# simonkosina/vbt

Hardware: AMD Instinct MI355X
Metric: frames/sec end-to-end (detect+NMS+track), EfficientDet-Lite0 320x320 (higher is better)
Workload: dtype int8

## Files before the change

vbt_amd/csrc/detector.hip:

```cpp
#include <algorithm>
#include <cmath>
#include <chrono>
#include <functional>
#include <map>
#include <set>
#include <type_traits>
#include <tuple>

#include "launchers.h"

namespace vbt {

static thread_local char g_err[512] = "";
void set_error(const char* fmt, ...) {
  va_list ap;
  va_start(ap, fmt);
  vsnprintf(g_err, sizeof(g_err), fmt, ap);
  va_end(ap);
}

bool lds_opt_in(const void* fn, LdsOptIn* state) {
  int dev = 0;
  if (hipGetDevice(&dev) != hipSuccess || dev < 0 || dev >= 64) { set_error("lds_opt_in: no current HIP device"); return false; }
  if (state->dev[dev] > 0) return true;
// ... 320 lines not shown
};
static FusedPlan resolve_fused(const vbt_model* m, const Step& s, int variant, int B) {
  const FusedArgs& a = s.fa;
  const OpRec& dop = m->ops[s.d_op];
  const int k = dop.k, stride = dop.stride;
  const bool ex = s.family == F_MBCONV, ks12 = a.KSe == 1 || a.KSe == 2;
  int var = variant;
  if (var < 0) {
    var = ((m->flags & VBT_MODEL_IMAGE_BLOCKS) && !resolve_fused(m, s, 5, B).rc) ? 5 : ((m->flags & VBT_MODEL_CHUNK48) ? 9 : 1);
    const FusedPlan p17 = (m->flags & VBT_MODEL_TILE128) ? resolve_fused(m, s, 17, B) : FusedPlan{};
    if (!p17.rc && p17.L.ppw2) var |= 16;
  }
  const bool mdw = var & 1, half = var & 2;
  const bool nt3 = (var & 8) && mdw && a.nch3 > 0 && s.nbp <= 2 && a.KSe >= 1 && a.KSe <= 4;
  FusedPlan p;
  if (var & 4) {
    const int HW = a.H * a.W, OHW = a.OH * a.OW;
    if (!ex || HW > 400 || OHW > 400 || !s.ib.data) { p.refuse(VBT_ERR_ARG, "fused_mbconv: whole-image variant not applicable"); return p; }
    p.image = true;
    p.PH = std::max((a.OH - 1) * stride + k, a.pad_t + a.H);
    p.PW = std::max((a.OW - 1) * stride + k, a.pad_l + a.W);
    p.NB = (a.Cout + 63) / 64;
    const int NPGo = (OHW + 15) / 16;
    const int units = (NPGo * p.NB + IB_WAVES - 1) / IB_WAVES;
    p.maxu = units <= 2 ? 2 : units <= 3 ? 3 : 4;
    p.L.k = k; p.L.stride = stride; p.L.lds_bytes = ((HW * a.T0S + 15) & ~15) + p.PH * p.PW * FB_EST + NPGo * 16 * FB_DST + s.ib.bytes;
    if (units > 4 || p.L.lds_bytes > 160 * 1024 || s.ib.bytes > 16 * IB_NPF * IB_THREADS) p.refuse(VBT_ERR_ARG, "fused_mbconv: whole-image variant not applicable");
    return p;
  }
  p.TX = a.TX;
  p.TY = half && a.TY >= 2 ? (a.TY + 1) / 2 : a.TY;
  const bool ppw2 = (var & 16) && ex && mdw && ks12 && s.nbp <= 2 && !half;
  if (ppw2) { p.TX = 16; p.TY = 8; }
  const bool dw64 = ppw2 || (ex && mdw && a.wd64 && p.TX == 8 && p.TY == 8 && ks12 && s.nbp <= 2);
  const int est = !ex ? 0 : !nt3 ? FB_EST : dw64 ? 48 : 72;
  p.tiles_x = (a.OW + p.TX - 1) / p.TX;
  p.tiles_y = (a.OH + p.TY - 1) / p.TY;
  p.L = FusedLaunch{k, stride, s.nbp, ex, mdw, nt3, ppw2, dw64, fused_tile_lds(a, k, stride, p.TX, p.TY, est, ppw2 ? 2 : 1, s.nbp),
                    (unsigned)((long)B * p.tiles_x * p.tiles_y)};
  if (ppw2 && (a.OW < 16 || a.OH < 8 || !a.wd64)) p.refuse(VBT_ERR_ARG, "fused_mbconv: the 128-pixel variant needs maps of at least 16 x 8");
  else if (ppw2 && p.L.lds_bytes > 64 * 1024) p.refuse(VBT_ERR_ARG, "fused_mbconv: 128-pixel tile needs %d bytes of LDS", p.L.lds_bytes);
  return p;
}
static int launch_fused_step(const vbt_model* m, const Step& s, FusedArgs a, int B, hipStream_t st) {
  const FusedPlan p = resolve_fused(m, s, s.variant, B);
  if (p.rc) return p.report();
  if (p.image) return launch_mbconv_image(a, s.ib, p.L.k, p.L.stride, p.maxu, p.PW, p.PH, p.NB, p.L.lds_bytes, B, st);
  a.TX = p.TX; a.TY = p.TY; a.tiles_x = p.tiles_x; a.tiles_y = p.tiles_y;
  return launch_fused_block(a, p.L, st);
}

struct ExpDwLaunch : Verdict {
  bool second = false; int cpw = 1, nw = 0, gpw = 0, lds = 0; unsigned grid = 0;
};
static ExpDwLaunch resolve_expdw(const vbt_model*, const Step& s, int variant, int B) {
  static const int xd_force = getenv("VBT_XD_VARIANT") ? atoi(getenv("VBT_XD_VARIANT")) : -100;
// ... 260 lines not shown
    cand = {0};
    for (int r : {1, 2, 4, 8, 16})
      if (r <= m->tensors[op.output].h) cand.push_back(r);
    if (m->tensors[op.output].c % 8 == 0) { cand.push_back(100); cand.push_back(101); }
  } else if (st.family == F_PW && st.KS64 <= 4) {
    cand = {0, 1};
  } else if (st.family == F_PW) {
    cand = {-1, 2, 3, 4, 5, 6};
  } else if (is_fused_tile(st.family)) {
    cand = {0, 1, 3, 5};
    if (st.family == F_MBCONV && st.fa.nch3 > 0 && st.nbp <= 2 && st.fa.KSe >= 1 && st.fa.KSe <= 4) { cand.push_back(9); cand.push_back(11); }
    if (st.family == F_MBCONV && st.nbp <= 2 && (st.fa.KSe == 1 || st.fa.KSe == 2)) {
      cand.push_back(17);
      if (st.fa.nch3 > 0) cand.push_back(25);
    }
  } else if (st.family == F_MULTI) {
    cand = {0, 1};
  } else if (st.family == F_EXPDW) {
    cand.clear();
    for (int cpw : {1, 2, 3, 4, 6})
      if (cpw <= st.xd.nchunks) cand.push_back(cpw);
    if (st.xd2_ok)
      for (int cpw : {1, 2, 3, 4, 6})
        if (cpw <= st.xd.nchunks) {
          if (st.xd2_gpw > 0) cand.push_back(100 + cpw);
          if (st.xd2_gpw16 > 0) cand.push_back(200 + cpw);
        }
  } else if (st.family == F_BAND) {
    cand = {-1, 0, 1};
  }
// ... 46 lines not shown
  }
  (void)hipDeviceSynchronize();
}

static PlanShape plan_shape(const vbt_model* m) {
  PlanShape shape;
  for (const Group& g : m->groups) {
    std::vector<std::vector<PlanStepShape>> alts;
    for (const Alt& a : g.alts) {
      std::vector<PlanStepShape> steps;
      for (const Step& st : a.steps) {
        PlanStepShape ps;
        ps.family = kFamilyName[st.family];
        ps.variants = candidate_variants(m, st);
        auto add = [&](int v) { if (std::find(ps.variants.begin(), ps.variants.end(), v) == ps.variants.end()) ps.variants.push_back(v); };
        for (int v = 0; v < 32 && is_fused_tile(st.family); v++)
          if (variant_ok(m, st, v)) add(v);
        add(-1);
        add(st.variant);
        steps.push_back(ps);
      }
      alts.push_back(steps);
    }
    shape.groups.push_back(alts);
  }
  return shape;
}
static bool load_plan(vbt_model* m, const char* path) {
  const PlanShape shape = plan_shape(m);
  std::vector<PlanChoice> sel;
  std::string note;
// ... 630 lines not shown
```

vbt_amd/csrc/dev_common.h:

```cpp
#pragma once
#include "common.h"

namespace vbt {

typedef int v4i __attribute__((ext_vector_type(4)));

__device__ __forceinline__ int requant(int acc, float mult, int zp, int lo, int hi) {
  float t = (float)acc * mult;
  t = fminf(fmaxf(t, -65536.0f), 65536.0f);
  int q = (int)__builtin_rintf(t) + zp;
  return min(max(q, lo), hi);
}
__device__ __forceinline__ unsigned pack4(int a, int b, int c, int d) {
  return (unsigned)(a & 255) | ((unsigned)(b & 255) << 8) | ((unsigned)(c & 255) << 16) | ((unsigned)(d & 255) << 24);
}

struct Rq {
  float lo_f, hi_f, off;
  int full;
  int kb;
};
constexpr int RQ_KBIAS = 0x4B400000;
__host__ __device__ inline Rq make_rq(int zp, int lo, int hi, int kb = 0) {
  return Rq{(float)(lo - zp), (float)(hi - zp), (float)(zp + 128), (lo <= -128 && hi >= 127) ? 1 : 0, kb};
// ... 30 lines not shown
    v2f r0 = (t0 + magic) + back;
    v2f r1 = (t1 + magic) + back;
    return pack4_u8f(r0.x, r0.y, r1.x, r1.y);
  }
  v2f r0 = {__builtin_amdgcn_fmed3f(__builtin_rintf(t0.x), q.lo_f, q.hi_f), __builtin_amdgcn_fmed3f(__builtin_rintf(t0.y), q.lo_f, q.hi_f)};
  v2f r1 = {__builtin_amdgcn_fmed3f(__builtin_rintf(t1.x), q.lo_f, q.hi_f), __builtin_amdgcn_fmed3f(__builtin_rintf(t1.y), q.lo_f, q.hi_f)};
  r0 = r0 + off;
  r1 = r1 + off;
  return pack4_u8f(r0.x, r0.y, r1.x, r1.y);
}
__device__ __forceinline__ v4i diag_operand(unsigned wb, int i) {
  const unsigned sh = wb << (8 * (i & 3));
  const int d = i >> 2;
  return (v4i){d == 0 ? (int)sh : 0, d == 1 ? (int)sh : 0, d == 2 ? (int)sh : 0, d == 3 ? (int)sh : 0};
}
__device__ __forceinline__ int fdiv_small(int n, float rcp_d) { return (int)(((float)n + 0.5f) * rcp_d); }
__device__ __forceinline__ float frcp(int d) { return __builtin_amdgcn_rcpf((float)d); }
__device__ __forceinline__ v4i v4i_from(const int4& b) { return (v4i){b.x, b.y, b.z, b.w}; }
__device__ __forceinline__ int4 int4_plus(const int4& b, int k) { return make_int4(b.x + k, b.y + k, b.z + k, b.w + k); }
template <class F>
__device__ __forceinline__ void rq_dispatch(const Rq& q, F&& f) {
  if (q.kb) { if (q.full) f(std::integral_constant<int, 3>{}); else f(std::integral_constant<int, 2>{}); }
  else { if (q.full) f(std::integral_constant<int, 1>{}); else f(std::integral_constant<int, 0>{}); }
}

__device__ __forceinline__ unsigned rq_pack_i(const v4i& acc, const int4& b, const float4& mu, const Rq& q) {
  const v4i a2 = {acc[0] + b.x, acc[1] + b.y, acc[2] + b.z, acc[3] + b.w};
  return rq_pack_b(a2, mu, q);
}

// ... 52 lines not shown
```

vbt_amd/csrc/expdw2_block.h:

```cpp
#pragma once
#include <type_traits>

#ifdef VBT_XD_PROF
#define XD2_STAMP(k) do { if (tid == 0) a.prof[(long)blockIdx.x * 32 + (k)] = __builtin_amdgcn_s_memtime(); } while (0)
#else
#define XD2_STAMP(k) do { } while (0)
#endif


struct ExpDw2Args {
  const int8_t* x;
  int8_t* out;
  int H, W, Cin, OH, OW, Ce;
  int pad_t, pad_l;
  int nchunks, cpw;
  int nbands, brows;
  int XB;
  int EQS, EYS;
  int e_bytes;
  int PS;
  int pe_off;
  int pd_off;
  const v4i* pe;
  const v4i* pd;
  Rq rqe;
  unsigned zeb;
  Rq rqd;
#ifdef VBT_XD_PROF
  unsigned long long* prof;
#endif
};

__device__ __forceinline__ v4i toeplitz_operand(unsigned w4, int c) {
  const int sh = 8 * c;
  return (v4i){(int)((w4 & 0xffu) << sh), (int)(((w4 >> 8) & 0xffu) << sh), (int)(((w4 >> 16) & 0xffu) << sh), (int)((w4 >> 24) << sh)};
}

constexpr int XD2_NPG = 8;
template <int PG, class F, class FC>
__device__ __forceinline__ void d_pair(F& d_units, FC full_c, int NPGo) {
  if constexpr (PG < XD2_NPG) {
    if (PG + 1 < NPGo) d_units(full_c, std::integral_constant<int, 2>{}, std::integral_constant<int, PG>{});
    else if (PG < NPGo) d_units(full_c, std::integral_constant<int, 1>{}, std::integral_constant<int, PG>{});
    if (PG + 2 < NPGo) d_pair<PG + 2>(d_units, full_c, NPGo);
  }
}

template <int KK, int S, int KS64, int NW, int GPW>
__global__ __launch_bounds__(64 * NW) void expdw2_kernel(ExpDw2Args a) {
  constexpr int DY = S, DX = 4 / S;
  constexpr int XD2_THREADS = 64 * NW, HW2 = NW / 2, QW = 16 / NW;
// ... 188 lines not shown
```

vbt_amd/csrc/fused_block.h:

```cpp
#pragma once

struct FusedArgs {
  const int8_t* x;
  int8_t* out;
  int H, W, Cin, OH, OW, Cout;
  int pad_t, pad_l;
  int TX, TY, tiles_x, tiles_y;
  int T0S;
  int nchunks;
  int zx;
  const long* we;
  const int* be;
  const float* me;
  int KSe, ze, loe, hie;
  Rq rqe;
  const long* we3;
  const long* wdm3;
  const v4i* wp3;
  int nch3, KSp3;
  const float* wd;
  const int* bd;
  const float* md;
  int zd, lod, hid;
  Rq rqd;
  const long* wdm;
  const int* bdm;
  const v4i* wd64;
  const long* wd64c;
  const v4i* wp;
  const int* bp;
  const float* mp;
  int KSp, zo, lop, hip;
  Rq rqp;
  int has_res;
  AddQ resq;
  int n_src;
  const int8_t* src[3];
  int sh[3], sw[3], smode[3], spt[3], spl[3];
  int chain;
  AddQ sumq, preq;
};

__device__ __forceinline__ unsigned node_sum4(const unsigned u[3], const FusedArgs& a) {
// ... 4 lines not shown

typedef unsigned short v2u16 __attribute__((ext_vector_type(2)));
__device__ __forceinline__ unsigned pk_max_u16(unsigned a, unsigned b) {
  v2u16 x, y;
  __builtin_memcpy(&x, &a, 4);
  __builtin_memcpy(&y, &b, 4);
  v2u16 r = __builtin_elementwise_max(x, y);
  unsigned o;
  __builtin_memcpy(&o, &r, 4);
  return o;
}

constexpr int FB_EST = 80;
constexpr int FB_DST = 80;

template <int KK, int S, int NBP, bool EXPAND, bool MDW, int KSE = 0, int NT = 4, int PPW = 1, bool DW64 = false>
__device__ __forceinline__ void fused_block_body(const FusedArgs& a, int tile, unsigned char* fb_smem) {
  static_assert(PPW == 1 || MDW, "128-pixel tiles exist for the matrix-pipe depthwise only");
  static_assert(!DW64 || (EXPAND && MDW && (KK == 3 || KK == 5)), "DW64: fused expand blocks, 3x3 / 5x5");
  const int tid = threadIdx.x, wave = tid >> 6, lane = tid & 63, r = lane & 15, g = lane >> 4;
  const int trow = fdiv_small(tile, frcp(a.tiles_x));
  const int tx = tile - trow * a.tiles_x;
  const int bimg = fdiv_small(trow, frcp(a.tiles_y));
  const int ty = trow - bimg * a.tiles_y;
  const long b = bimg;
  const int oy0 = ty * a.TY, ox0 = tx * a.TX;
  const int TXp = (a.TX + 3) & ~3;
  const int HWx = (TXp - 1) * S + KK, HWy = (a.TY - 1) * S + KK, NPh = HWx * HWy;
  const int iy0 = oy0 * S - a.pad_t, ix0 = ox0 * S - a.pad_l;
  const float rcp_hwx = frcp(HWx), rcp_txp = frcp(TXp);
  unsigned char* T0 = fb_smem;
  unsigned char* E = T0 + ((NPh * a.T0S + 15) & ~15);
  constexpr int EST = (EXPAND && NT == 3) ? (DW64 ? 48 : 72) : FB_EST;
  unsigned char* D = E + (EXPAND ? ((NPh * EST + 15) & ~15) : 0);
  bool stage_p = false;
  if constexpr (!EXPAND && NBP <= 2) stage_p = a.nchunks == 1;
  unsigned char* WPS = D + 64 * PPW * FB_DST;
  unsigned char* BPS = WPS + NBP * 4096;

  bool summed = false;
  if constexpr (!EXPAND) summed = a.n_src > 0;
  if (summed) {
    const int nd = a.Cin >> 2;
    const unsigned zb4 = (unsigned)(a.zx & 255) * 0x01010101u;
    const int pstep = fdiv_small(256, frcp(nd));
    int p = fdiv_small(tid, frcp(nd));
    const int cd = tid - p * nd;
    const bool up2[3] = {a.H == 2 * a.sh[0] && a.W == 2 * a.sw[0], a.H == 2 * a.sh[1] && a.W == 2 * a.sw[1], a.H == 2 * a.sh[2] && a.W == 2 * a.sw[2]};
    for (; tid < pstep * nd && p < NPh; p += pstep) {
// ... 107 lines not shown
  const int nsx = TXp >> 2;
  const int sy = fdiv_small(strip, frcp(nsx)), sx = (strip - sy * nsx) * 4;
  const bool dw_active = sy < a.TY;
  int hbase[4 * PPW];
#pragma unroll
  for (int pg = 0; pg < 4 * PPW; pg++) hbase[pg] = 0;
  if constexpr (MDW && !DW64) {
#pragma unroll
    for (int pg = 0; pg < 4 * PPW; pg++) {
      int slot = pg * 16 + r;
      int sq = TXp == 8 ? (slot >> 3) : fdiv_small(slot, rcp_txp);
      int py_ = min(sq, a.TY - 1), px_ = slot - sq * TXp;
      hbase[pg] = (py_ * S) * HWx + px_ * S;
    }
  }
  constexpr int KTP = (KK * KK + 1) / 2;
  long wpre[KTP];
  int4 bpre = make_int4(0, 0, 0, 0);
  float4 mpre = make_float4(0.f, 0.f, 0.f, 0.f);
  if constexpr (!EXPAND && MDW) {
    const long* wm0 = a.wdm + ((long)wave * KTP) * 64 + lane;
#pragma unroll
    for (int mi = 0; mi < KTP; mi++) wpre[mi] = wm0[mi * 64];
    bpre = *(const int4*)(a.bdm + 16 * wave + 4 * g);
    mpre = *(const float4*)(a.md + 16 * wave + 4 * g);
  }
  __syncthreads();

  constexpr int CH = 16 * NT;
  const int nch = NT == 3 ? a.nch3 : a.nchunks;
  const long* const wdm_ = NT == 3 ? a.wdm3 : a.wdm;
  for (int c = 0; c < nch; c++) {
    constexpr bool PREF_DW = EXPAND && MDW && KSE >= 3;
    if constexpr (PREF_DW) {
      if (NT == 4 || wave < NT) {
        const long* wmc = wdm_ + ((long)(c * NT + wave) * KTP) * 64 + lane;
#pragma unroll
        for (int mi = 0; mi < KTP; mi++) wpre[mi] = wmc[mi * 64];
        bpre = *(const int4*)(a.bdm + c * CH + 16 * wave + 4 * g);
        mpre = *(const float4*)(a.md + c * CH + 16 * wave + 4 * g);
      }
    }
    if (EXPAND) {
      int4 eb[NT];
      float4 em[NT];
#pragma unroll
      for (int t = 0; t < NT; t++) {
        eb[t] = *(const int4*)(a.be + c * CH + 4 * NT * g + 4 * t);
        em[t] = *(const float4*)(a.me + c * CH + 4 * NT * g + 4 * t);
      }
      const unsigned zeb = (unsigned)(a.ze & 255) * 0x01010101u;
      const long* w = (NT == 3 ? a.we3 : a.we) + (long)c * a.KSe * NT * 64 + lane;
      long wreg[KSE > 0 ? KSE : 1][NT];
      if constexpr (KSE > 0) {
#pragma unroll
        for (int ks = 0; ks < KSE; ks++)
#pragma unroll
// ... 21 lines not shown
          } else {
#pragma unroll 2
            for (int ks = 0; ks < a.KSe; ks++) {
              long bv = *(const long*)(brow + 32 * ks);
#pragma unroll
              for (int t = 0; t < NT; t++) ea[t] = __builtin_amdgcn_mfma_i32_16x16x32_i8(w[(ks * NT + t) * 64], bv, ea[t], 0, 0, 0);
            }
          }
          unsigned d[NT];
#pragma unroll
          for (int t = 0; t < NT; t++) {
            d[t] = rq_pack_b<FULLK>(ea[t], em[t], a.rqe);
            if ((oob_mask >> i) & 1u) d[t] = zeb;
          }
          if (!((tail_mask >> i) & 1u)) {
            if constexpr (NT == 4) {
              *(uint4*)(E + p * FB_EST + 16 * g) = make_uint4(d[0], d[1], d[2], d[3]);
            } else {
#pragma unroll
              for (int t = 0; t < NT; t++) *(unsigned*)(E + p * EST + 4 * NT * g + 4 * t) = d[t];
            }
          }
        }
      };
      rq_dispatch(a.rqe, expand_loop);
      __syncthreads();
    }
    if constexpr (DW64) {
      constexpr int TXP = 8 * PPW, HWX = (TXP - 1) * S + KK;
      constexpr int KT64 = KK == 3 ? 3 : 7;
      constexpr int PGS = (16 / TXP) * S * HWX * EST;
      if (NT == 4 || wave < NT) {
        const unsigned long long wc = (unsigned long long)a.wd64c[(long)(c * NT + wave) * 64 + lane];
        v4i wreg[KT64];
#pragma unroll
        for (int mi = 0; mi < KT64; mi++) wreg[mi] = diag_operand((unsigned)(wc >> (8 * mi)) & 0xffu, r);
        const int4 bq0 = *(const int4*)(a.bdm + c * CH + 16 * wave + 4 * g);
        const float4 mum = *(const float4*)(a.md + c * CH + 16 * wave + 4 * g);
        const int hb = TXP == 8 ? ((r >> 3) * S * HWX + (r & 7) * S) : r * S;
        const unsigned char* baseH = E + hb * EST + 16 * wave + g * EST;
        const unsigned char* baseV = E + hb * EST + 16 * wave + g * (HWX * EST);
        auto dw_walk = [&](auto mode_tag) {
          constexpr int RM = decltype(mode_tag)::value;
// ... 91 lines not shown
        }
      }
      const int4 bq = *(const int4*)(a.bd + c * 64 + 4 * cq);
      const float4 mu = *(const float4*)(a.md + c * 64 + 4 * cq);
#pragma unroll
      for (int o = 0; o < 4; o++) {
        v4i ai = {(int)dacc[o][0], (int)dacc[o][1], (int)dacc[o][2], (int)dacc[o][3]};
        unsigned dd = rq_pack_i(ai, bq, mu, a.rqd);
        *(unsigned*)(D + (sy * TXp + sx + o) * FB_DST + 4 * cq) = dd;
      }
    }
    __syncthreads();
    {
      v4i bv[PPW];
#pragma unroll
      for (int pp = 0; pp < PPW; pp++) bv[pp] = *(const v4i*)(D + ((wave * PPW + pp) * 16 + r) * FB_DST + 16 * g);
#pragma unroll
      for (int nb = 0; nb < NBP; nb++) {
        const v4i* w = stage_p ? (const v4i*)WPS + (nb * 4) * 64 + lane
                               : (NT == 3 ? a.wp3 + ((long)(nb * a.KSp3 + c) * 4) * 64 : a.wp + ((long)(nb * a.KSp + c) * 4) * 64) + lane;
#pragma unroll
        for (int t = 0; t < 4; t++) {
          const v4i wv = w[t * 64];
#pragma unroll
          for (int pp = 0; pp < PPW; pp++) acc[pp][nb][t] = __builtin_amdgcn_mfma_i32_16x16x64_i8(wv, bv[pp], acc[pp][nb][t], 0, 0, 0);
        }
      }
    }
    if (!EXPAND && c + 1 < nch) __syncthreads();
  }

// ... 39 lines not shown
#pragma unroll
        for (int t = 0; t < 4; t++)
#pragma unroll
          for (int j = 0; j < 4; j++)
            if (c0 + 4 * t + j < a.Cout) o[4 * t + j] = (int8_t)(d[t] >> (8 * j));
      }
    }
  }
  }
}


#ifndef FB_MINW
#define FB_MINW 1
#endif
template <int KK, int S, int NBP, bool EXPAND, bool MDW, int KSE = 0, int NT = 4, int PPW = 1, bool DW64 = false>
__global__ __launch_bounds__(256, FB_MINW) void fused_block_kernel(FusedArgs a) {
  extern __shared__ __attribute__((aligned(16))) unsigned char fb_smem_dyn[];
  fused_block_body<KK, S, NBP, EXPAND, MDW, KSE, NT, PPW, DW64>(a, blockIdx.x, fb_smem_dyn);
}

struct MultiTiles {
  int n;
  int start[13];
};
template <int KK, int S, int NBP, bool EXPAND, bool MDW>
__global__ __launch_bounds__(256, FB_MINW) void fused_block_multi_kernel(const FusedArgs* __restrict__ args, MultiTiles mt) {
  extern __shared__ __attribute__((aligned(16))) unsigned char fb_smem_dyn[];
  int p = 0;
#pragma unroll
  for (int i = 1; i < 12; i++)
    if (i < mt.n && (int)blockIdx.x >= mt.start[i]) p = i;
  fused_block_body<KK, S, NBP, EXPAND, MDW>(args[p], (int)blockIdx.x - mt.start[p], fb_smem_dyn);
}
// ... 138 lines not shown
```

vbt_amd/csrc/k_fused_mbconv.hip:

```cpp
#include "launchers.h"

namespace vbt {

#define FB_P2(KK, S, NBP, KSE)                                                                                      \
  do {                                                                                                              \
    if (L.nt3) fused_block_kernel<KK, S, NBP, true, true, KSE, 3, 2, true><<<grid, 256, L.lds_bytes, st>>>(a);      \
    else fused_block_kernel<KK, S, NBP, true, true, KSE, 4, 2, true><<<grid, 256, L.lds_bytes, st>>>(a);            \
  } while (0)
#define FB_P2K(KK, S)                                                                                               \
  do {                                                                                                              \
    if (L.nbp == 1 && a.KSe == 1) FB_P2(KK, S, 1, 1);                                                               \
    else if (L.nbp == 1) FB_P2(KK, S, 1, 2);                                                                        \
    else if (a.KSe == 1) FB_P2(KK, S, 2, 1);                                                                        \
    else FB_P2(KK, S, 2, 2);                                                                                        \
  } while (0)
#define FB_DW64(KK, S, NBP)                                                                                                                    \
  do {                                                                                                                                         \
    if (L.nt3 && a.KSe == 1) fused_block_kernel<KK, S, (NBP <= 2 ? NBP : 1), true, true, 1, 3, 1, true><<<grid, 256, L.lds_bytes, st>>>(a);    \
    else if (L.nt3) fused_block_kernel<KK, S, (NBP <= 2 ? NBP : 1), true, true, 2, 3, 1, true><<<grid, 256, L.lds_bytes, st>>>(a);            \
    else if (a.KSe == 1) fused_block_kernel<KK, S, (NBP <= 2 ? NBP : 1), true, true, 1, 4, 1, true><<<grid, 256, L.lds_bytes, st>>>(a);       \
    else fused_block_kernel<KK, S, (NBP <= 2 ? NBP : 1), true, true, 2, 4, 1, true><<<grid, 256, L.lds_bytes, st>>>(a);                       \
  } while (0)
#define FB_LAUNCH(KK, S, NBP)                                                                                                                          \
  do {                                                                                                                                                 \
// ... 7 lines not shown
    else if (L.mdw && a.KSe == 3) fused_block_kernel<KK, S, NBP, true, true, 3><<<grid, 256, L.lds_bytes, st>>>(a);                                   \
    else if (L.mdw && a.KSe == 4) fused_block_kernel<KK, S, NBP, true, true, 4><<<grid, 256, L.lds_bytes, st>>>(a);                                   \
    else if (L.mdw) fused_block_kernel<KK, S, NBP, true, true><<<grid, 256, L.lds_bytes, st>>>(a);                                                    \
    else fused_block_kernel<KK, S, NBP, true, false><<<grid, 256, L.lds_bytes, st>>>(a);                                                              \
  } while (0)
#define FB_NBP(KK, S)                                      \
  do {                                                     \
    switch (L.nbp) {                                       \
      case 1: FB_LAUNCH(KK, S, 1); break;                  \
      case 2: FB_LAUNCH(KK, S, 2); break;                  \
      case 3: FB_LAUNCH(KK, S, 3); break;                  \
      default: FB_LAUNCH(KK, S, 5); break;                 \
    }                                                      \
  } while (0)

int launch_fused_mbconv(const FusedArgs& a, const FusedLaunch& L, hipStream_t st) {
  const dim3 grid(L.grid);
  if (L.ppw2) {
    if (L.k == 3 && L.stride == 1) FB_P2K(3, 1);
    else if (L.k == 3 && L.stride == 2) FB_P2K(3, 2);
    else if (L.k == 5 && L.stride == 1) FB_P2K(5, 1);
    else FB_P2K(5, 2);
    return VBT_OK;
  }
  if (L.k == 3 && L.stride == 1) FB_NBP(3, 1);
  else if (L.k == 3 && L.stride == 2) FB_NBP(3, 2);
  else if (L.k == 5 && L.stride == 1) FB_NBP(5, 1);
  else FB_NBP(5, 2);
  return VBT_OK;
}

// ... 2 lines not shown
```

vbt_amd/csrc/launchers.h:

```cpp
#pragma once
#include "dev_common.h"

namespace vbt {
#include "fused_block.h"
#include "stem_block.h"
#include "image_block.h"
#include "expdw_block.h"
#include "expdw2_block.h"
#include "band_block.h"

struct FusedLaunch {
  int k, stride, nbp;
  bool expand;
  bool mdw;
  bool nt3;
  bool ppw2;
  bool dw64;
  int lds_bytes;
  unsigned grid;
};
int launch_fused_block(const FusedArgs& a, const FusedLaunch& L, hipStream_t st);
int launch_fused_multi(const FusedArgs* d_args, const MultiTiles& mt, int k, int stride, int nbp, bool mdw, int lds_bytes, unsigned grid,
                       hipStream_t st);
int launch_dw_tile(const DwTileArgs& a, int k, int stride, bool mdw, dim3 grid, int lds_bytes, hipStream_t st);
int launch_mbconv_image(const FusedArgs& a, const ImageBundle& wb, int k, int stride, int maxu, int PW, int PH, int NB, int lds_bytes, int B,
                        hipStream_t st);
int launch_band_one(const BandArgs& a, bool chained, unsigned grid, int lds_bytes, hipStream_t st);
int launch_band_multi(const BandArgs* d_probs, const MultiTiles& mt, int C, bool chained, unsigned grid, int lds_bytes, hipStream_t st);
int launch_expdw(const ExpDwArgs& a, int k, int stride, int KS64, unsigned grid, int lds_bytes, hipStream_t st);
int launch_expdw2(const ExpDw2Args& a, int k, int stride, int KS64, int nw, int gpw, unsigned grid, int lds_bytes, hipStream_t st);
int launch_stem_block(const StemBlockArgs& a, bool full_range, unsigned grid, hipStream_t st);

}
```

vbt_amd/csrc/planner.h:

```cpp
#pragma once

static int conv_kb(const vbt_model* m, const OpRec& op) {
  const bool off = getenv("VBT_NO_KBIAS") != nullptr;
  if (off || (op.type != OP_STEM && op.type != OP_PW && op.type != OP_DW)) return 0;
  const TensorRec& tin = m->tensors[op.inputs[0]];
  const TensorRec& tout = m->tensors[op.output];
  const int8_t* w = (const int8_t*)(m->blob.data() + op.w_off);
  const int32_t* bq = (const int32_t*)(m->blob.data() + op.b_off);
  const bool dw = op.type == OP_DW;
  const int N = tout.c, K = dw ? op.k * op.k : op.k * op.k * tin.c;
  for (int co = 0; co < N; co++) {
    long long sa = 0;
    for (int k = 0; k < K; k++) sa += std::abs((int)(dw ? w[(size_t)k * N + co] : w[(size_t)co * K + k]));
    if (255 * sa + std::llabs((long long)bq[co]) >= (1ll << 22) - 1) return 0;
  }
  return 1;
}

static void choose_tile(int OH, int OW, int KK, int S, bool expand, int* TXo, int* TYo, int slots = 64) {
  double best = 1e300;
  for (int TX = 1; TX <= std::min(OW, 64); TX++) {
    int TXp = (TX + 3) & ~3;
    int TY = std::min(OH, slots / TXp);
    if (TY < 1) continue;
    int tiles = ((OW + TX - 1) / TX) * ((OH + TY - 1) / TY);
    int NPh = ((TXp - 1) * S + KK) * ((TY - 1) * S + KK);
    double cost = tiles * ((expand ? 1.0 : 0.35) * NPh + (double)slots);
    if (cost < best) { best = cost; *TXo = TX; *TYo = TY; }
  }
}

static int fused_tile_lds(const FusedArgs& a, int k, int stride, int TX, int TY, int est, int ppw, int nbp) {
  const int TXp = (TX + 3) & ~3;
  const int NPh = ((TXp - 1) * stride + k) * ((TY - 1) * stride + k);
  int lds = ((NPh * a.T0S + 15) & ~15) + ((NPh * est + 15) & ~15) + ppw * 64 * FB_DST;
  if (!est && a.nchunks == 1 && nbp <= 2) lds += nbp * (4096 + 512);
  return lds;
}

struct NodeSrc { int n = 0; int tensor[3]; int mode[3]; int rs_op[3] = {-1, -1, -1}; int pre_add = -1; int chain = 0; };

static Cost cost_of(const vbt_model* m, std::initializer_list<int> ops, const NodeSrc* ns = nullptr) {
  Cost c;
  for (int oi : ops)
    if (oi >= 0) c += m->op_steps[oi].cost;
  if (ns) c += cost_of(m, {ns->rs_op[0], ns->rs_op[1], ns->rs_op[2], ns->pre_add});
  return c;
}

template <typename Args>
// ... 94 lines not shown
  }
  {
    float* dwf; int* dbias; float* dmult;
    if ((rc = upload(m, dw_weights_f32(wd, Ce, kk, Cp), &dwf)) || (rc = upload(m, fold_bias(bqd, wd, Ce, kk, 128 + tdin.zero_point, W_TAPS, Cp), &dbias)) ||
        (rc = upload(m, pad_floats((const float*)(m->blob.data() + dop.m_off), Ce, Cp), &dmult)))
      return rc;
    a.wd = dwf; a.bd = dbias; a.md = dmult;
    long* dwdm; int* dbm;
    if ((rc = upload(m, pack_dw_diag(wd, Ce, kk, 64), &dwdm)) || (rc = upload(m, fold_bias(bqd, wd, Ce, kk, tdin.zero_point, W_TAPS, Cp), &dbm))) return rc;
    a.wdm = dwdm; a.bdm = dbm;
    if (expand && (dop.k == 3 || dop.k == 5)) {
      const std::vector<v4i> w64 = pack_dw64(wd, Ce, dop.k, Cp / 16);
      v4i* d64; long* d64c;
      if ((rc = upload(m, w64, &d64)) || (rc = upload(m, pack_dw64_compact(w64, dop.k), &d64c))) return rc;
      a.wd64 = d64; a.wd64c = d64c;
    }
    a.zd = tdout.zero_point; a.lod = dop.act_min; a.hid = dop.act_max;
    a.rqd = make_rq(a.zd, a.lod, a.hid, conv_kb(m, dop));
  }
  {
    std::vector<v4i> wp;
    pack_weights64(wpj, tout.c, Ce, Cp / 64, s.nbp, wp);
    v4i* dwp;
    if ((rc = upload(m, wp, &dwp))) return rc;
    a.wp = dwp; a.bp = ps.bias; a.mp = ps.mult; a.KSp = Cp / 64;
    a.zo = tout.zero_point; a.lop = pop.act_min; a.hip = pop.act_max;
    a.rqp = make_rq(a.zo, a.lop, a.hip);
  }
  if (a_op >= 0) {
    a.has_res = 1;
// ... 373 lines not shown
  if ((rc = upload(m, pe, &dpe)) || (rc = upload(m, pack_expdw_taps(wd, Ce, kk), &dpd)) || (rc = upload(m, be, &dbe)) || (rc = upload(m, bd, &dbd)) ||
      (rc = upload(m, me, &dme)) || (rc = upload(m, md, &dmd)))
    return rc;
  a.we = dpe; a.wdc = dpd; a.be = dbe; a.bd = dbd; a.me = dme; a.md = dmd;
  a.rqe = make_rq(te.zero_point, eop.act_min, eop.act_max, conv_kb(m, eop));
  a.rqd = make_rq(td.zero_point, dop.act_min, dop.act_max, conv_kb(m, dop));
  a.zeb = (unsigned)(te.zero_point & 255) * 0x01010101u;
  s.lds_bytes = geo.t0_bytes + geo.e_bytes + geo.d_bytes;
  s.cost = cost_of(m, {e_op, d_op});
  if ((rc = make_expdw2(m, e_op, d_op, &s, pe, be, me, bd, md))) return rc;
  *out = s;
  return VBT_OK;
}

static long xd2_read_cycles(int PR, int XB, int EYS, int RM) {
  static const int grp[4][16] = {{0, 1, 2, 3, 12, 13, 14, 15, 20, 21, 22, 23, 24, 25, 26, 27},
                                 {4, 5, 6, 7, 8, 9, 10, 11, 16, 17, 18, 19, 28, 29, 30, 31},
                                 {32, 33, 34, 35, 44, 45, 46, 47, 52, 53, 54, 55, 56, 57, 58, 59},
                                 {36, 37, 38, 39, 40, 41, 42, 43, 48, 49, 50, 51, 60, 61, 62, 63}};
  const int NPOS = PR * XB;
  long cycles = 0;
  for (int pg = 0; pg * 16 < NPOS; pg++)
    for (int k = 0; k < 4; k++) {
      std::vector<int> seen[16];
      int worst = 1;
      for (int j = 0; j < 16; j++) {
        const int lane = grp[k][j], r = lane & 15, g = lane >> 4, n = std::min(pg * 16 + r, NPOS - 1);
        const int addr = (n / XB) * RM * EYS + (n % XB) * 16 + (g >> 1) * EYS + 16 * (g & 1);
        std::vector<int>& v = seen[(addr >> 4) & 15];
        if (std::find(v.begin(), v.end(), addr) == v.end()) v.push_back(addr);
        worst = std::max(worst, (int)v.size());
      }
      cycles += worst;
    }
  return cycles;
}
struct ExpDw2Geom { bool ok; int nbands, brows, XB, EQS, EYS, e_bytes, PS, pe_off, pd_off, lds, gpw, gpw16; };
static ExpDw2Geom expdw2_geom(int H, int W, int OH, int OW, int k, int stride, int pad_t, int KS64, int nbands) {
  ExpDw2Geom g{};
  const int DY = stride, DX = 4 / stride;
  g.brows = (OH + nbands - 1) / nbands;
  if (DY == 2) g.brows = (g.brows + 1) & ~1;
// ... 55 lines not shown
  a.pad_t = a1.pad_t; a.pad_l = a1.pad_l;
  a.nchunks = a1.nchunks; a.cpw = 1; a.nbands = geo.nbands; a.brows = geo.brows;
  a.XB = geo.XB; a.EQS = geo.EQS; a.EYS = geo.EYS; a.e_bytes = geo.e_bytes; a.PS = geo.PS; a.pe_off = geo.pe_off; a.pd_off = geo.pd_off;
  a.rqe = a1.rqe; a.zeb = a1.zeb; a.rqd = a1.rqd;
  const TensorRec& te = m->tensors[m->ops[e_op].output];
  const int Ce = te.c, nch = a.nchunks, kk = dop.k, S = dop.stride, KT2 = (S * (S - 1) + kk + 1) / 2;
  const int NE = KS64 * 256 + 32, ND = KT2 * 256 + 32;
  const int8_t* wd = (const int8_t*)(m->blob.data() + dop.w_off);
  std::vector<v4i> ppe((size_t)nch * NE), ppd((size_t)nch * ND);
  for (int c = 0; c < nch; c++) {
    v4i* e = &ppe[(size_t)c * NE];
    memcpy(e, &pe[(size_t)c * KS64 * 256], sizeof(v4i) * KS64 * 256);
    memcpy(e + KS64 * 256, &be[c * 64], 256);
    memcpy(e + KS64 * 256 + 16, &me[c * 64], 256);
    v4i* d = &ppd[(size_t)c * ND];
    const std::vector<unsigned> tab = pack_expdw2_taps(wd, Ce, c, kk, S);
    memcpy(d, tab.data(), tab.size() * sizeof(unsigned));
    memcpy(d + KT2 * 256, &bd[c * 64], 256);
    memcpy(d + KT2 * 256 + 16, &md[c * 64], 256);
  }
  v4i *dpe, *dpd;
  int rc;
  if ((rc = upload(m, ppe, &dpe)) || (rc = upload(m, ppd, &dpd))) return rc;
  a.pe = dpe; a.pd = dpd;
  s->xd2_ok = true;
  s->xd2_lds = geo.lds;
  s->xd2_gpw = geo.gpw;
  s->xd2_gpw16 = geo.gpw16;
  return VBT_OK;
}

// ... 467 lines not shown
```

vbt_amd/csrc/weight_pack.h:

```cpp
#pragma once

static void pack_weights(const int8_t* w, int N, int K, int KS, int NB, const std::vector<int>* kmap, std::vector<long>& out) {
  out.assign((size_t)NB * KS * 4 * 64, 0);
  int8_t* o = (int8_t*)out.data();
  for (int nb = 0; nb < NB; nb++)
    for (int ks = 0; ks < KS; ks++)
      for (int t = 0; t < 4; t++)
        for (int lane = 0; lane < 64; lane++) {
          int i = lane & 15, g = lane >> 4;
          int co = 64 * nb + 16 * (i >> 2) + 4 * t + (i & 3);
          for (int j = 0; j < 8; j++) {
            int kp = 32 * ks + 8 * g + j;
            int k = kmap ? (kp < (int)kmap->size() ? (*kmap)[kp] : -1) : (kp < K ? kp : -1);
            int8_t v = (co < N && k >= 0) ? w[(size_t)co * K + k] : 0;
            o[((((size_t)(nb * KS + ks) * 4 + t) * 64 + lane) * 8) + j] = v;
          }
        }
}

static void pack_weights64(const int8_t* w, int N, int K, int KS, int NB, std::vector<v4i>& out, const std::vector<int>* kmap = nullptr) {
  out.assign((size_t)NB * KS * 4 * 64, (v4i){0, 0, 0, 0});
  int8_t* o = (int8_t*)out.data();
  for (int nb = 0; nb < NB; nb++)
    for (int ks = 0; ks < KS; ks++)
// ... 188 lines not shown
  return out;
}
static std::vector<long> pack_expdw_taps(const int8_t* w, int Ce, int kk) {
  const int nch = (Ce + 63) / 64, KT = (kk + 3) / 4;
  std::vector<long> out((size_t)nch * 4 * 64, 0);
  int8_t* o = (int8_t*)out.data();
  for (int c = 0; c < nch; c++)
    for (int cg = 0; cg < 4; cg++)
      for (int mi = 0; mi < KT; mi++)
        for (int lane = 0; lane < 64; lane++) {
          const int i = lane & 15, g = lane >> 4, ch = 64 * c + 16 * cg + i, tap = 4 * mi + g;
          o[(((size_t)(c * 4 + cg)) * 64 + lane) * 8 + mi] = (tap < kk && ch < Ce) ? w[(size_t)tap * Ce + ch] : 0;
        }
  return out;
}
static std::vector<unsigned> pack_expdw2_taps(const int8_t* w, int Ce, int c, int k, int S) {
  const int KT2 = (S * (S - 1) + k + 1) / 2;
  std::vector<unsigned> out((size_t)16 * KT2 * 64, 0);
  for (int q = 0; q < 16; q++)
    for (int mi = 0; mi < KT2; mi++)
      for (int lane = 0; lane < 64; lane++) {
        const int i = lane & 15, g = lane >> 4, qq = i >> 2, cc = i & 3, ch = 64 * c + 4 * q + cc;
        const int dy = S == 2 ? qq >> 1 : 0, dx = S == 2 ? qq & 1 : qq;
        const int ty = 2 * mi + (g >> 1) - S * dy;
        unsigned w4 = 0;
        for (int j = 0; j < 4; j++) {
          const int tx = 4 * (g & 1) + j - S * dx;
          if (ty >= 0 && ty < k && tx >= 0 && tx < k && ch < Ce) w4 |= (unsigned)(uint8_t)w[(size_t)(ty * k + tx) * Ce + ch] << (8 * j);
        }
        out[(q * KT2 + mi) * 64 + lane] = w4;
      }
  return out;
}
```

Before: 118,300.

## Add Toeplitz-matrix depthwise variant to fused MBConv tile kernel

Adds a new fused MBConv variant (bit 32) that computes the depthwise convolution as Toeplitz-packed int8 MFMA products. The expand stage writes into a new LDS layout chosen to reduce bank conflicts, and the depthwise output uses a skewed slot mapping. Weights are pre-packed per step at plan time. The autotuner gains candidates 33/41/49/57, so the variant only runs where tuning picks it. The cost is extra weight uploads, more kernel instantiations, and extra complexity in the LDS layout.

Result: faster. 119,600 (median of 6 runs) (+1.1%).

```diff
diff --git a/vbt_amd/csrc/detector.hip b/vbt_amd/csrc/detector.hip
--- a/vbt_amd/csrc/detector.hip
+++ b/vbt_amd/csrc/detector.hip
@@ -358,6 +358,7 @@
   const bool mdw = var & 1, half = var & 2;
   const bool nt3 = (var & 8) && mdw && a.nch3 > 0 && s.nbp <= 2 && a.KSe >= 1 && a.KSe <= 4;
   FusedPlan p;
+  if ((var & 32) && (var & 4)) { p.refuse(VBT_ERR_ARG, "fused_mbconv: variant %d: the Toeplitz depthwise does not apply to this step", var); return p; }
   if (var & 4) {
     const int HW = a.H * a.W, OHW = a.OH * a.OW;
     if (!ex || HW > 400 || OHW > 400 || !s.ib.data) { p.refuse(VBT_ERR_ARG, "fused_mbconv: whole-image variant not applicable"); return p; }
@@ -378,12 +379,18 @@
   if (ppw2) { p.TX = 16; p.TY = 8; }
   const bool dw64 = ppw2 || (ex && mdw && a.wd64 && p.TX == 8 && p.TY == 8 && ks12 && s.nbp <= 2);
   const int est = !ex ? 0 : !nt3 ? FB_EST : dw64 ? 48 : 72;
+  const bool tpz = var & 32;
+  const bool tpz_ok = tpz && dw64 && a.wtz && fused_tpz_built(k, stride, s.nbp, a.KSe, ppw2) && (var & ~(1 | 8 | 16 | 32)) == 0 && nt3 == bool(var & 8) && ppw2 == bool(var & 16);
+  const TpzGeom tg = tpz_ok ? tpz_geom(k, stride, ppw2 ? 2 : 1, nt3 ? 3 : 4) : TpzGeom{};
+  const int e_bytes = tpz_ok ? tg.e_bytes + 8 * tg.DSK : -1;
   p.tiles_x = (a.OW + p.TX - 1) / p.TX;
   p.tiles_y = (a.OH + p.TY - 1) / p.TY;
-  p.L = FusedLaunch{k, stride, s.nbp, ex, mdw, nt3, ppw2, dw64, fused_tile_lds(a, k, stride, p.TX, p.TY, est, ppw2 ? 2 : 1, s.nbp),
-                    (unsigned)((long)B * p.tiles_x * p.tiles_y)};
+  p.L = FusedLaunch{k, stride, s.nbp, ex, mdw, nt3, ppw2, dw64, fused_tile_lds(a, k, stride, p.TX, p.TY, est, ppw2 ? 2 : 1, s.nbp, e_bytes),
+                    (unsigned)((long)B * p.tiles_x * p.tiles_y), tpz_ok};
   if (ppw2 && (a.OW < 16 || a.OH < 8 || !a.wd64)) p.refuse(VBT_ERR_ARG, "fused_mbconv: the 128-pixel variant needs maps of at least 16 x 8");
   else if (ppw2 && p.L.lds_bytes > 64 * 1024) p.refuse(VBT_ERR_ARG, "fused_mbconv: 128-pixel tile needs %d bytes of LDS", p.L.lds_bytes);
+  else if (tpz && !tpz_ok) p.refuse(VBT_ERR_ARG, "fused_mbconv: variant %d: the Toeplitz depthwise does not apply to this step", var);
+  else if (tpz && p.L.lds_bytes > 64 * 1024) p.refuse(VBT_ERR_ARG, "fused_mbconv: the Toeplitz depthwise tile needs %d bytes of LDS", p.L.lds_bytes);
   return p;
 }
 static int launch_fused_step(const vbt_model* m, const Step& s, FusedArgs a, int B, hipStream_t st) {
@@ -674,6 +681,7 @@
       cand.push_back(17);
       if (st.fa.nch3 > 0) cand.push_back(25);
     }
+    if (st.family == F_MBCONV && st.fa.wtz) cand.insert(cand.end(), {33, 41, 49, 57});
   } else if (st.family == F_MULTI) {
     cand = {0, 1};
   } else if (st.family == F_EXPDW) {
@@ -750,7 +758,7 @@
         ps.family = kFamilyName[st.family];
         ps.variants = candidate_variants(m, st);
         auto add = [&](int v) { if (std::find(ps.variants.begin(), ps.variants.end(), v) == ps.variants.end()) ps.variants.push_back(v); };
-        for (int v = 0; v < 32 && is_fused_tile(st.family); v++)
+        for (int v = 0; v < 64 && is_fused_tile(st.family); v++)
           if (variant_ok(m, st, v)) add(v);
         add(-1);
         add(st.variant);
diff --git a/vbt_amd/csrc/dev_common.h b/vbt_amd/csrc/dev_common.h
--- a/vbt_amd/csrc/dev_common.h
+++ b/vbt_amd/csrc/dev_common.h
@@ -68,6 +68,10 @@
   const int d = i >> 2;
   return (v4i){d == 0 ? (int)sh : 0, d == 1 ? (int)sh : 0, d == 2 ? (int)sh : 0, d == 3 ? (int)sh : 0};
 }
+__device__ __forceinline__ v4i toeplitz_operand(unsigned w4, int c) {
+  const int sh = 8 * c;
+  return (v4i){(int)((w4 & 0xffu) << sh), (int)(((w4 >> 8) & 0xffu) << sh), (int)(((w4 >> 16) & 0xffu) << sh), (int)((w4 >> 24) << sh)};
+}
 __device__ __forceinline__ int fdiv_small(int n, float rcp_d) { return (int)(((float)n + 0.5f) * rcp_d); }
 __device__ __forceinline__ float frcp(int d) { return __builtin_amdgcn_rcpf((float)d); }
 __device__ __forceinline__ v4i v4i_from(const int4& b) { return (v4i){b.x, b.y, b.z, b.w}; }
diff --git a/vbt_amd/csrc/expdw2_block.h b/vbt_amd/csrc/expdw2_block.h
--- a/vbt_amd/csrc/expdw2_block.h
+++ b/vbt_amd/csrc/expdw2_block.h
@@ -30,11 +30,6 @@
   unsigned long long* prof;
 #endif
 };
-
-__device__ __forceinline__ v4i toeplitz_operand(unsigned w4, int c) {
-  const int sh = 8 * c;
-  return (v4i){(int)((w4 & 0xffu) << sh), (int)(((w4 >> 8) & 0xffu) << sh), (int)(((w4 >> 16) & 0xffu) << sh), (int)((w4 >> 24) << sh)};
-}
 
 constexpr int XD2_NPG = 8;
 template <int PG, class F, class FC>
diff --git a/vbt_amd/csrc/fused_block.h b/vbt_amd/csrc/fused_block.h
--- a/vbt_amd/csrc/fused_block.h
+++ b/vbt_amd/csrc/fused_block.h
@@ -1,4 +1,5 @@
 #pragma once
+#include "tpz_geom.h"
 
 struct FusedArgs {
   const int8_t* x;
@@ -27,6 +28,7 @@
   const int* bdm;
   const v4i* wd64;
   const long* wd64c;
+  const unsigned* wtz;
   const v4i* wp;
   const int* bp;
   const float* mp;
@@ -61,10 +63,13 @@
 constexpr int FB_EST = 80;
 constexpr int FB_DST = 80;
 
-template <int KK, int S, int NBP, bool EXPAND, bool MDW, int KSE = 0, int NT = 4, int PPW = 1, bool DW64 = false>
+template <int KK, int S, int NBP, bool EXPAND, bool MDW, int KSE = 0, int NT = 4, int PPW = 1, bool DW64 = false, bool TPZ = false>
 __device__ __forceinline__ void fused_block_body(const FusedArgs& a, int tile, unsigned char* fb_smem) {
   static_assert(PPW == 1 || MDW, "128-pixel tiles exist for the matrix-pipe depthwise only");
   static_assert(!DW64 || (EXPAND && MDW && (KK == 3 || KK == 5)), "DW64: fused expand blocks, 3x3 / 5x5");
+  static_assert(!TPZ || (DW64 && (S == 1 || S == 2) && (NT == 3 || NT == 4) && NBP <= 2 && (KSE == 1 || KSE == 2)), "TPZ: a form of DW64");
+  constexpr TpzGeom TG = TPZ ? tpz_geom(KK, S, PPW, NT) : TpzGeom{};
+  constexpr int KT2 = (S * (S - 1) + KK + 1) / 2;
   const int tid = threadIdx.x, wave = tid >> 6, lane = tid & 63, r = lane & 15, g = lane >> 4;
   const int trow = fdiv_small(tile, frcp(a.tiles_x));
   const int tx = tile - trow * a.tiles_x;
@@ -79,7 +84,7 @@
   unsigned char* T0 = fb_smem;
   unsigned char* E = T0 + ((NPh * a.T0S + 15) & ~15);
   constexpr int EST = (EXPAND && NT == 3) ? (DW64 ? 48 : 72) : FB_EST;
-  unsigned char* D = E + (EXPAND ? ((NPh * EST + 15) & ~15) : 0);
+  unsigned char* D = E + (EXPAND ? (TPZ ? TG.e_bytes : ((NPh * EST + 15) & ~15)) : 0);
   bool stage_p = false;
   if constexpr (!EXPAND && NBP <= 2) stage_p = a.nchunks == 1;
   unsigned char* WPS = D + 64 * PPW * FB_DST;
@@ -217,6 +222,12 @@
       hbase[pg] = (py_ * S) * HWx + px_ * S;
     }
   }
+  const int wq0 = TPZ ? __builtin_amdgcn_readfirstlane(wave) * NT : 0;
+  int tz_e = 0, tz_d = 0;
+  if constexpr (TPZ) {
+    tz_e = tpz_e_offset(TG, S, r, g, wq0);
+    tz_d = tpz_d_offset(TG, S, PPW, FB_DST, r, g, wq0);
+  }
   constexpr int KTP = (KK * KK + 1) / 2;
   long wpre[KTP];
   int4 bpre = make_int4(0, 0, 0, 0);
@@ -244,6 +255,12 @@
         mpre = *(const float4*)(a.md + c * CH + 16 * wave + 4 * g);
       }
     }
+    unsigned wtz[TPZ ? NT * KT2 : 1];
+    if constexpr (TPZ) {
+      const unsigned* wt = a.wtz + ((long)(c * 4 * NT + wq0) * KT2) * 64 + lane;
+#pragma unroll
+      for (int i = 0; i < NT * KT2; i++) wtz[i] = wt[i * 64];
+    }
     if (EXPAND) {
       int4 eb[NT];
       float4 em[NT];
@@ -295,7 +312,12 @@
             if ((oob_mask >> i) & 1u) d[t] = zeb;
           }
           if (!((tail_mask >> i) & 1u)) {
-            if constexpr (NT == 4) {
+            if constexpr (TPZ) {
+              const int hy = fdiv_small(p, rcp_hwx), hx = p - hy * HWx;
+              unsigned char* ep = E + tpz_e_store(TG, hy, hx, NT * g);
+#pragma unroll
+              for (int t = 0; t < NT; t++) *(unsigned*)(ep + t * TG.EQS) = d[t];
+            } else if constexpr (NT == 4) {
               *(uint4*)(E + p * FB_EST + 16 * g) = make_uint4(d[0], d[1], d[2], d[3]);
             } else {
 #pragma unroll
@@ -307,7 +329,43 @@
       rq_dispatch(a.rqe, expand_loop);
       __syncthreads();
     }
-    if constexpr (DW64) {
+    if constexpr (TPZ) {
+      constexpr int NU = NT * PPW, PGE = tpz_e_group(TG, S), PGD = tpz_d_group(TG, PPW, FB_DST);
+      int4 bq[NT];
+      float4 mq[NT];
+#pragma unroll
+      for (int q = 0; q < NT; q++) {
+        bq[q] = *(const int4*)(a.bdm + c * CH + 4 * (wq0 + q));
+        mq[q] = *(const float4*)(a.md + c * CH + 4 * (wq0 + q));
+      }
+      const unsigned char* eb = E + tz_e;
+      unsigned char* db = D + tz_d;
+      auto tz_walk = [&](auto mode_tag) {
+        constexpr int RM = decltype(mode_tag)::value;
+#pragma unroll
+        for (int u0 = 0; u0 < NU; u0 += 2) {
+          v4i dq[2];
+#pragma unroll
+          for (int u = 0; u < 2; u++) dq[u] = v4i_from(int4_plus(bq[(u0 + u < NU ? u0 + u : u0) / PPW], RM >= 2 ? RQ_KBIAS : 0));
+#pragma unroll
+          for (int mi = 0; mi < KT2; mi++)
+#pragma unroll
+            for (int u = 0; u < 2; u++) {
+              if (u0 + u >= NU) continue;
+              const int q = (u0 + u) / PPW, pg = (u0 + u) % PPW;
+              const v4i bv = *(const v4i*)(eb + q * TG.EQS + pg * PGE + mi * 2 * TG.EYS);
+              dq[u] = __builtin_amdgcn_mfma_i32_16x16x64_i8(toeplitz_operand(wtz[q * KT2 + mi], r & 3), bv, dq[u], 0, 0, 0);
+            }
+#pragma unroll
+          for (int u = 0; u < 2; u++) {
+            if (u0 + u >= NU) continue;
+            const int q = (u0 + u) / PPW, pg = (u0 + u) % PPW;
+            *(unsigned*)(db + pg * PGD + 4 * q) = rq_pack_b<RM>(dq[u], mq[q], a.rqd);
+          }
+        }
+      };
+      rq_dispatch(a.rqd, tz_walk);
+    } else if constexpr (DW64) {
       constexpr int TXP = 8 * PPW, HWX = (TXP - 1) * S + KK;
       constexpr int KT64 = KK == 3 ? 3 : 7;
       constexpr int PGS = (16 / TXP) * S * HWX * EST;
@@ -429,7 +487,10 @@
     {
       v4i bv[PPW];
 #pragma unroll
-      for (int pp = 0; pp < PPW; pp++) bv[pp] = *(const v4i*)(D + ((wave * PPW + pp) * 16 + r) * FB_DST + 16 * g);
+      for (int pp = 0; pp < PPW; pp++) {
+        const int slot = (wave * PPW + pp) * 16 + r;
+        bv[pp] = *(const v4i*)(D + (TPZ ? tpz_d_slot(TG, PPW, FB_DST, slot) : slot * FB_DST) + 16 * g);
+      }
 #pragma unroll
       for (int nb = 0; nb < NBP; nb++) {
         const v4i* w = stage_p ? (const v4i*)WPS + (nb * 4) * 64 + lane
@@ -499,10 +560,10 @@
 #ifndef FB_MINW
 #define FB_MINW 1
 #endif
-template <int KK, int S, int NBP, bool EXPAND, bool MDW, int KSE = 0, int NT = 4, int PPW = 1, bool DW64 = false>
+template <int KK, int S, int NBP, bool EXPAND, bool MDW, int KSE = 0, int NT = 4, int PPW = 1, bool DW64 = false, bool TPZ = false>
 __global__ __launch_bounds__(256, FB_MINW) void fused_block_kernel(FusedArgs a) {
   extern __shared__ __attribute__((aligned(16))) unsigned char fb_smem_dyn[];
-  fused_block_body<KK, S, NBP, EXPAND, MDW, KSE, NT, PPW, DW64>(a, blockIdx.x, fb_smem_dyn);
+  fused_block_body<KK, S, NBP, EXPAND, MDW, KSE, NT, PPW, DW64, TPZ>(a, blockIdx.x, fb_smem_dyn);
 }
 
 struct MultiTiles {
diff --git a/vbt_amd/csrc/k_fused_mbconv.hip b/vbt_amd/csrc/k_fused_mbconv.hip
--- a/vbt_amd/csrc/k_fused_mbconv.hip
+++ b/vbt_amd/csrc/k_fused_mbconv.hip
@@ -45,7 +45,10 @@
     }                                                      \
   } while (0)
 
+int launch_fused_mbconv_tpz(const FusedArgs& a, const FusedLaunch& L, hipStream_t st);
+
 int launch_fused_mbconv(const FusedArgs& a, const FusedLaunch& L, hipStream_t st) {
+  if (L.tpz) return launch_fused_mbconv_tpz(a, L, st);
   const dim3 grid(L.grid);
   if (L.ppw2) {
     if (L.k == 3 && L.stride == 1) FB_P2K(3, 1);
diff --git a/vbt_amd/csrc/k_fused_mbconv_tpz.hip b/vbt_amd/csrc/k_fused_mbconv_tpz.hip
--- /dev/null
+++ b/vbt_amd/csrc/k_fused_mbconv_tpz.hip
@@ -0,0 +1,32 @@
+#include "launchers.h"
+
+namespace vbt {
+
+#define FB_TPZ1(KK, S, NBP, KSE)                                                                                 \
+  do {                                                                                                                            \
+    if (L.nt3) fused_block_kernel<KK, S, NBP, true, true, KSE, 3, 1, true, true><<<grid, 256, L.lds_bytes, st>>>(a);              \
+    else fused_block_kernel<KK, S, NBP, true, true, KSE, 4, 1, true, true><<<grid, 256, L.lds_bytes, st>>>(a);                    \
+    return VBT_OK;                                                                                                                \
+  } while (0)
+#define FB_TPZ2(KK, S, NBP, KSE)                                                                                \
+  do {                                                                                                                            \
+    if (L.nt3) fused_block_kernel<KK, S, NBP, true, true, KSE, 3, 2, true, true><<<grid, 256, L.lds_bytes, st>>>(a);              \
+    else fused_block_kernel<KK, S, NBP, true, true, KSE, 4, 2, true, true><<<grid, 256, L.lds_bytes, st>>>(a);                    \
+    return VBT_OK;                                                                                                                \
+  } while (0)
+#define FB_TPZ(KK, S, NBP, KSE) do { if (L.ppw2) FB_TPZ2(KK, S, NBP, KSE); else FB_TPZ1(KK, S, NBP, KSE); } while (0)
+
+int launch_fused_mbconv_tpz(const FusedArgs& a, const FusedLaunch& L, hipStream_t st) {
+  const dim3 grid(L.grid);
+  const int k = L.k, s = L.stride, nbp = L.nbp, kse = a.KSe;
+  if (L.dw64 && a.wtz && fused_tpz_built(k, s, nbp, kse, L.ppw2)) {
+    if (k == 3 && s == 2 && nbp == 1 && kse == 1) FB_TPZ(3, 2, 1, 1);
+    if (k == 3 && s == 1 && nbp == 1 && kse == 1) FB_TPZ(3, 1, 1, 1);
+    if (k == 5 && s == 2 && nbp == 1 && kse == 1) FB_TPZ1(5, 2, 1, 1);
+    if (k == 5 && s == 1 && nbp == 1 && kse == 2) FB_TPZ(5, 1, 1, 2);
+  }
+  set_error("fused_mbconv: no Toeplitz-depthwise instantiation for k=%d s=%d nbp=%d KSe=%d%s", k, s, nbp, kse, L.ppw2 ? " on 16 x 8 tiles" : "");
+  return VBT_ERR_ARG;
+}
+
+}
diff --git a/vbt_amd/csrc/launchers.h b/vbt_amd/csrc/launchers.h
--- a/vbt_amd/csrc/launchers.h
+++ b/vbt_amd/csrc/launchers.h
@@ -18,7 +18,12 @@
   bool dw64;
   int lds_bytes;
   unsigned grid;
+  bool tpz = false;
 };
+static inline bool fused_tpz_built(int k, int stride, int nbp, int kse, bool ppw2) {
+  return (k == 3 && stride == 2 && nbp == 1 && kse == 1) || (k == 3 && stride == 1 && nbp == 1 && kse == 1) ||
+         (k == 5 && stride == 2 && nbp == 1 && kse == 1 && !ppw2) || (k == 5 && stride == 1 && nbp == 1 && kse == 2);
+}
 int launch_fused_block(const FusedArgs& a, const FusedLaunch& L, hipStream_t st);
 int launch_fused_multi(const FusedArgs* d_args, const MultiTiles& mt, int k, int stride, int nbp, bool mdw, int lds_bytes, unsigned grid,
                        hipStream_t st);
diff --git a/vbt_amd/csrc/planner.h b/vbt_amd/csrc/planner.h
--- a/vbt_amd/csrc/planner.h
+++ b/vbt_amd/csrc/planner.h
@@ -30,10 +30,10 @@
   }
 }
 
-static int fused_tile_lds(const FusedArgs& a, int k, int stride, int TX, int TY, int est, int ppw, int nbp) {
+static int fused_tile_lds(const FusedArgs& a, int k, int stride, int TX, int TY, int est, int ppw, int nbp, int e_bytes = -1) {
   const int TXp = (TX + 3) & ~3;
   const int NPh = ((TXp - 1) * stride + k) * ((TY - 1) * stride + k);
-  int lds = ((NPh * a.T0S + 15) & ~15) + ((NPh * est + 15) & ~15) + ppw * 64 * FB_DST;
+  int lds = ((NPh * a.T0S + 15) & ~15) + (e_bytes >= 0 ? e_bytes : ((NPh * est + 15) & ~15)) + ppw * 64 * FB_DST;
   if (!est && a.nchunks == 1 && nbp <= 2) lds += nbp * (4096 + 512);
   return lds;
 }
@@ -158,6 +158,11 @@
       v4i* d64; long* d64c;
       if ((rc = upload(m, w64, &d64)) || (rc = upload(m, pack_dw64_compact(w64, dop.k), &d64c))) return rc;
       a.wd64 = d64; a.wd64c = d64c;
+      if (fused_tpz_built(dop.k, dop.stride, s.nbp, a.KSe, false)) {
+        unsigned* dtz;
+        if ((rc = upload(m, pack_expdw2_taps(wd, Ce, 0, Cp / 4, dop.k, dop.stride), &dtz))) return rc;
+        a.wtz = dtz;
+      }
     }
     a.zd = tdout.zero_point; a.lod = dop.act_min; a.hid = dop.act_max;
     a.rqd = make_rq(a.zd, a.lod, a.hid, conv_kb(m, dop));
@@ -561,10 +566,6 @@
 }
 
 static long xd2_read_cycles(int PR, int XB, int EYS, int RM) {
-  static const int grp[4][16] = {{0, 1, 2, 3, 12, 13, 14, 15, 20, 21, 22, 23, 24, 25, 26, 27},
-                                 {4, 5, 6, 7, 8, 9, 10, 11, 16, 17, 18, 19, 28, 29, 30, 31},
-                                 {32, 33, 34, 35, 44, 45, 46, 47, 52, 53, 54, 55, 56, 57, 58, 59},
-                                 {36, 37, 38, 39, 40, 41, 42, 43, 48, 49, 50, 51, 60, 61, 62, 63}};
   const int NPOS = PR * XB;
   long cycles = 0;
   for (int pg = 0; pg * 16 < NPOS; pg++)
@@ -572,7 +573,7 @@
       std::vector<int> seen[16];
       int worst = 1;
       for (int j = 0; j < 16; j++) {
-        const int lane = grp[k][j], r = lane & 15, g = lane >> 4, n = std::min(pg * 16 + r, NPOS - 1);
+        const int lane = DS_READ_B128_GROUPS[k][j], r = lane & 15, g = lane >> 4, n = std::min(pg * 16 + r, NPOS - 1);
         const int addr = (n / XB) * RM * EYS + (n % XB) * 16 + (g >> 1) * EYS + 16 * (g & 1);
         std::vector<int>& v = seen[(addr >> 4) & 15];
         if (std::find(v.begin(), v.end(), addr) == v.end()) v.push_back(addr);
@@ -658,7 +659,7 @@
     memcpy(e + KS64 * 256, &be[c * 64], 256);
     memcpy(e + KS64 * 256 + 16, &me[c * 64], 256);
     v4i* d = &ppd[(size_t)c * ND];
-    const std::vector<unsigned> tab = pack_expdw2_taps(wd, Ce, c, kk, S);
+    const std::vector<unsigned> tab = pack_expdw2_taps(wd, Ce, 64 * c, 16, kk, S);
     memcpy(d, tab.data(), tab.size() * sizeof(unsigned));
     memcpy(d + KT2 * 256, &bd[c * 64], 256);
     memcpy(d + KT2 * 256 + 16, &md[c * 64], 256);
diff --git a/vbt_amd/csrc/tpz_geom.h b/vbt_amd/csrc/tpz_geom.h
--- /dev/null
+++ b/vbt_amd/csrc/tpz_geom.h
@@ -0,0 +1,54 @@
+#pragma once
+
+struct TpzGeom { int XB, EQS, EYS, rows, e_bytes, DSK; };
+constexpr int DS_READ_B128_GROUPS[4][16] = {{0, 1, 2, 3, 12, 13, 14, 15, 20, 21, 22, 23, 24, 25, 26, 27},
+                                            {4, 5, 6, 7, 8, 9, 10, 11, 16, 17, 18, 19, 28, 29, 30, 31},
+                                            {32, 33, 34, 35, 44, 45, 46, 47, 52, 53, 54, 55, 56, 57, 58, 59},
+                                            {36, 37, 38, 39, 40, 41, 42, 43, 48, 49, 50, 51, 60, 61, 62, 63}};
+constexpr int tpz_position(int r) { return 2 * (r & 7) + (((r >> 2) & 1) ^ (((r + 4) >> 3) & 1)); }
+constexpr int tpz_read_cycles(int S, int XB, int npg, int EYS) {
+  int cycles = 0;
+  for (int pg = 0; pg < npg; pg++)
+    for (int k = 0; k < 4; k++) {
+      int seen[16][16] = {}, ns[16] = {}, worst = 1;
+      for (int j = 0; j < 16; j++) {
+        const int lane = DS_READ_B128_GROUPS[k][j], g = lane >> 4, n = pg * 16 + tpz_position(lane & 15);
+        const int addr = (n / XB) * S * S * EYS + (n % XB) * 16 + (g >> 1) * EYS + 16 * (g & 1), b = (addr >> 4) & 15;
+        bool dup = false;
+        for (int h = 0; h < ns[b]; h++) dup = dup || seen[b][h] == addr;
+        if (!dup) seen[b][ns[b]++] = addr;
+        if (ns[b] > worst) worst = ns[b];
+      }
+      cycles += worst;
+    }
+  return cycles;
+}
+constexpr TpzGeom tpz_geom(int KK, int S, int PPW, int NT) {
+  TpzGeom g{};
+  g.XB = 8 * PPW * S / 4;
+  g.EQS = 16 * (g.XB + 1);
+  const int KT2 = (S * (S - 1) + KK + 1) / 2;
+  g.rows = S * S * (8 / S - 1) + 2 * KT2;
+  int best = -1;
+  for (int pad = 0; pad < 256; pad += 16) {
+    const int cyc = tpz_read_cycles(S, g.XB, PPW, 4 * NT * g.EQS + pad);
+    if (best < 0 || cyc < best) { best = cyc; g.EYS = 4 * NT * g.EQS + pad; }
+  }
+  g.e_bytes = g.rows * g.EYS;
+  g.DSK = S == 1 ? 16 : 0;
+  return g;
+}
+
+constexpr int tpz_e_offset(const TpzGeom& G, int S, int r, int g, int q0) {
+  const int n = tpz_position(r), y = n / G.XB, xk = n % G.XB;
+  return (S * S * y + (g >> 1)) * G.EYS + 16 * xk + 16 * (g & 1) + q0 * G.EQS;
+}
+constexpr int tpz_e_group(const TpzGeom& G, int S) { return (16 / G.XB) * S * S * G.EYS; }
+constexpr int tpz_e_store(const TpzGeom& G, int hy, int hx, int q) { return hy * G.EYS + 4 * hx + q * G.EQS; }
+constexpr int tpz_d_slot(const TpzGeom& G, int PPW, int dst, int slot) { return slot * dst + (slot / (8 * PPW)) * G.DSK; }
+constexpr int tpz_d_offset(const TpzGeom& G, int S, int PPW, int dst, int r, int g, int q0) {
+  const int n = tpz_position(r), y = n / G.XB, xk = n % G.XB;
+  const int py = S == 1 ? y : 2 * y + (g >> 1), px = S == 1 ? 4 * xk + g : 2 * xk + (g & 1);
+  return tpz_d_slot(G, PPW, dst, py * 8 * PPW + px) + 4 * q0;
+}
+constexpr int tpz_d_group(const TpzGeom& G, int PPW, int dst) { return 64 * dst + (64 / (8 * PPW)) * G.DSK; }
diff --git a/vbt_amd/csrc/weight_pack.h b/vbt_amd/csrc/weight_pack.h
--- a/vbt_amd/csrc/weight_pack.h
+++ b/vbt_amd/csrc/weight_pack.h
@@ -226,13 +226,13 @@
         }
   return out;
 }
-static std::vector<unsigned> pack_expdw2_taps(const int8_t* w, int Ce, int c, int k, int S) {
+static std::vector<unsigned> pack_expdw2_taps(const int8_t* w, int Ce, int base, int nq, int k, int S) {
   const int KT2 = (S * (S - 1) + k + 1) / 2;
-  std::vector<unsigned> out((size_t)16 * KT2 * 64, 0);
-  for (int q = 0; q < 16; q++)
+  std::vector<unsigned> out((size_t)nq * KT2 * 64, 0);
+  for (int q = 0; q < nq; q++)
     for (int mi = 0; mi < KT2; mi++)
       for (int lane = 0; lane < 64; lane++) {
-        const int i = lane & 15, g = lane >> 4, qq = i >> 2, cc = i & 3, ch = 64 * c + 4 * q + cc;
+        const int i = lane & 15, g = lane >> 4, qq = i >> 2, cc = i & 3, ch = base + 4 * q + cc;
         const int dy = S == 2 ? qq >> 1 : 0, dx = S == 2 ? qq & 1 : qq;
         const int ty = 2 * mi + (g >> 1) - S * dy;
         unsigned w4 = 0;
@@ -240,7 +240,7 @@
           const int tx = 4 * (g & 1) + j - S * dx;
           if (ty >= 0 && ty < k && tx >= 0 && tx < k && ch < Ce) w4 |= (unsigned)(uint8_t)w[(size_t)(ty * k + tx) * Ce + ch] << (8 * j);
         }
-        out[(q * KT2 + mi) * 64 + lane] = w4;
-      }
-  return out;
-}
+        out[((size_t)q * KT2 + mi) * 64 + lane] = w4;
+      }
+  return out;
+}
```
